# aewallwi/calamity

Measured on AMD Instinct MI355X. Metric: Adam steps/sec (chi2 eval/sec in extra), HERA-350 1024ch DPSS; %HBM roofline, higher is better.
Workload: dtype f32; 1 GPU; hera350: 350 antennas, 61075 baselines x 1024 channels, per-baseline DPSS (sum nvec = 6080554) per time slice, 1 time slice(s), optimizer Adam lr 1e-2, model_regularization none; layout=stream, parallelism=single GPU

## Files before the change

### calamity_amd/csrc/calamity_hip.hip

```cpp
#include "../../include/calamity_hip.h"

#include <hip/hip_runtime.h>
#include <rccl/rccl.h>

#include <algorithm>
#include <cmath>
#include <cstdarg>
#include <cstdio>
#include <cstring>
#include <limits>
#include <map>
#include <memory>
#include <mutex>
#include <numeric>
#include <string>
#include <vector>

#include "fit_kernels.hpp"
#include "dense_kernels.hpp"
#include "split_kernels.hpp"
#include "split2_kernels.hpp"
#include "dense64_kernels.hpp"
#include "multi_mfma_kernels.hpp"
#include "gain_basis_kernels.hpp"
// ... 739 lines not shown
    if (t && nslices > 1) {
      for (int sl = 1; sl < nslices; ++sl)
        if (h_state[sl].t != h_state[0].t)
          return fail(CAL_ERR_STATE, "get_moments: the %d time slices of this solver have applied different numbers of updates (slice 0: %lld, slice %d: %lld); "
                      "one iteration count cannot resume them bit for bit", nslices, (long long)h_state[0].t, sl, (long long)h_state[sl].t);
    }
    if (gm_r) CAL_TRY(download_rows(gm_r, gains_m.as<T>(), nants, 2, 0));
    if (gm_i) CAL_TRY(download_rows(gm_i, gains_m.as<T>(), nants, 2, 1));
    if (gv_r) CAL_TRY(download_rows(gv_r, gains_v.as<T>(), nants, 2, 0));
    if (gv_i) CAL_TRY(download_rows(gv_i, gains_v.as<T>(), nants, 2, 1));
    const size_t cb = (size_t)ncoef * sizeof(T);
    if (cm_r) HIP_TRY(copy_sync(cm_r, coef_m.as<T>(), cb, hipMemcpyDeviceToHost));
    if (cm_i) HIP_TRY(copy_sync(cm_i, coef_m.as<T>() + ncoef, cb, hipMemcpyDeviceToHost));
    if (cv_r) HIP_TRY(copy_sync(cv_r, coef_v.as<T>(), cb, hipMemcpyDeviceToHost));
    if (cv_i) HIP_TRY(copy_sync(cv_i, coef_v.as<T>() + ncoef, cb, hipMemcpyDeviceToHost));
    if (t) *t = h_state->t;
    return CAL_OK;
  }

  int set_moments(const void* gm_r, const void* gm_i, const void* gv_r, const void* gv_i, const void* cm_r, const void* cm_i,
                  const void* cv_r, const void* cv_i, int64_t t) override {
    HIP_TRY(hipSetDevice(device));
    if (!has_problem) return fail(CAL_ERR_STATE, "set_moments before set_problem");
    if (tb_on()) return fail(CAL_ERR_UNSUPPORTED, "set_moments: checkpoint / resume of a fit with a gain time basis is not supported");
    if (gb_on()) return fail(CAL_ERR_UNSUPPORTED, "set_moments: checkpoint / resume of a fit with a gain basis is not supported");
    if (t < 0) return fail(CAL_ERR_INVALID, "set_moments: negative iteration count");
    if (gm_r) CAL_TRY(upload_rows(gm_r, gains_m.as<T>(), nants, 2, 0));
    if (gm_i) CAL_TRY(upload_rows(gm_i, gains_m.as<T>(), nants, 2, 1));
    if (gv_r) CAL_TRY(upload_rows(gv_r, gains_v.as<T>(), nants, 2, 0));
    if (gv_i) CAL_TRY(upload_rows(gv_i, gains_v.as<T>(), nants, 2, 1));
    const size_t cb = (size_t)ncoef * sizeof(T);
    if (cm_r) HIP_TRY(copy_sync(coef_m.as<T>(), cm_r, cb, hipMemcpyHostToDevice));
    if (cm_i) HIP_TRY(copy_sync(coef_m.as<T>() + ncoef, cm_i, cb, hipMemcpyHostToDevice));
    if (cv_r) HIP_TRY(copy_sync(coef_v.as<T>(), cv_r, cb, hipMemcpyHostToDevice));
    if (cv_i) HIP_TRY(copy_sync(coef_v.as<T>() + ncoef, cv_i, cb, hipMemcpyHostToDevice));
    double b1t = 1.0, b2t = 1.0, sched = 1.0;
    for (int64_t k = 0; k < t; ++k) {
      b1t *= opt.beta_1;
      b2t *= opt.beta_2;
    }
    if (opt.optimizer == CAL_OPT_NADAM && t > 0) {
      hipLaunchKernelGGL(nadam_sched_kernel, dim3(1), dim3(1), 0, stream, opt.beta_1, (long long)t, scal.as<double>());
      HIP_TRY(hipGetLastError());
      HIP_TRY(hipMemcpyAsync(&sched, scal.p, sizeof(double), hipMemcpyDeviceToHost, stream));
      HIP_TRY(hipStreamSynchronize(stream));
    }
    for (int sl = 0; sl < nslices; ++sl) {
      h_state[sl].t = t;
      h_state[sl].b1t = b1t;
      h_state[sl].b2t = b2t;
      h_state[sl].nadam_sched = sched;
    }
    return CAL_OK;
  }

  template <typename A> A pass_args() {
    A a{};
    a.data_r = data_r.as<T>();
    a.data_i = data_i.as<T>();
    a.wgts = wgts.as<T>();
    a.gains = gains.as<T2>();
    a.c_r = coef.as<T>();
    a.c_i = coef.as<T>() + ncoef;
    a.q0 = q0.as<T2>();
    a.part = part.as<double>();
    a.state = st_cur();
    a.nslices = nslices;
    a.fpad = fpad;
    a.nbls = nbls;
    return a;
  }
  FusedArgs<T> fused_args() {
    FusedArgs<T> a = pass_args<FusedArgs<T>>();
    a.tiles = tiles.as<T>();
    a.bl_tile = bl_tile.as<long long>();
    a.bl_ant = bl_ant.as<int2>();
    a.items = items.as<Item>();
    a.q1 = q1.as<T2>();
    a.gcp0_r = gcp0.as<T>();
    a.gcp0_i = gcp0.as<T>() + gcp_len;
    a.gcp1_r = gcp1.as<T>();
    a.gcp1_i = gcp1.p ? gcp1.as<T>() + gcp_len : nullptr;
    a.runs = runs.as<int2>();
    a.stream_once = layout == CAL_LAYOUT_STREAM ? 1 : 0;
    a.members = members.as<Member>();
    a.heads = nheads > 0 ? heads.as<int>() : nullptr;
    a.nfreqs = nfreqs;
    return a;
  }
  FusedArgs<T> model_args() {
    FusedArgs<T> a = fused_args();
    a.model_r = model_buf.as<T>();
    a.model_i = model_buf.as<T>() + (size_t)nbls * fpad;
    return a;
  }
  using DenseArgs = typename std::conditional<std::is_same<T, float>::value, MfmaArgs, Dense64Args>::type;
  DenseArgs dense_args() {
    DenseArgs m = pass_args<DenseArgs>();
    m.ops = mf_ops.as<T>();
    m.panels = mf_panels.as<PanelItem>();
    m.gc_r = grad_c0();
    m.gc_i = grad_c0() + ncoef;
    m.slot_map = mf_map.as<int>();
    return m;
  }
  StepShape step_shape(PassAsk ask, int nsteps = 0) const {
    return plan_step(StepInputs{mf_ok, reg == CAL_REG_SUM, reg_prepass, gc_direct, comm_on(), yb_on(), 2LL * nants * fpad + 2LL * ncoef <= (1LL << 20), launch_mode,
                                opt.optimizer == CAL_OPT_LAMB, ask, timing, nsteps >= kGraphMinSteps});
  }

  using FusedFn = void (*)(const FusedArgs<T>);
  static FusedFn pick(bool with_reg, FusedFn reg, FusedFn plain) { return with_reg ? reg : plain; }
  template <int MODE, int L> FusedFn basis_kernel(bool with_reg) const {
    return fold ? pick(with_reg, fused_basis_kernel<T, MODE, true, L, true>, fused_basis_kernel<T, MODE, false, L, true>)
                : pick(with_reg, fused_basis_kernel<T, MODE, true, L, false>, fused_basis_kernel<T, MODE, false, L, false>);
  }
  static constexpr size_t kQLdsMax1 = TileCfg<T, FbSet<T>::fb_min>::q_lds_bytes(false);
  static constexpr size_t kQLdsMax2 = TileCfg<T, FbSet<T>::fb_min>::q_lds_bytes(true);
  template <int MODE> void launch_fused(FusedArgs<T> a, bool with_reg) {
    constexpr bool kPass = MODE == MODE_LOSS || MODE == MODE_GRAD;
    const int nsimple = (kPass && nheads > 0) ? nitems_plain : nitems_simple;
    if (nsimple > 0) {
      FusedFn k = basis_kernel<MODE, kMaxLoads>(with_reg);
      if constexpr (kPass)
        if (small_loads) k = basis_kernel<MODE, kSmallLoads>(with_reg);
      const size_t lds = lds_bytes + (MODE == MODE_GRAD ? (with_reg ? kQLdsMax2 : kQLdsMax1) : 0);
      hipLaunchKernelGGL(k, dim3(nsimple), dim3(kThreads), lds, stream, a);
    }
    if constexpr (kPass) {
      if (nheads > 0) {
        if (nheads_mfma > 0) {
          FusedFn k = pick(with_reg, fused_multi_mfma_kernel<T, MODE, 1>, fused_multi_mfma_kernel<T, MODE, 0>);
          if (with_reg && MODE == MODE_GRAD && heads_one_pass) k = fused_multi_mfma_kernel<T, MODE_GRAD, 2>;
          hipLaunchKernelGGL(k, dim3(mm_grid), dim3(kThreads), lds_multi_mfma_bytes, stream, a);
        }
        if (nheads > nheads_mfma) {
          FusedArgs<T> b = a;
          b.heads = a.heads + mm_grid;
          const FusedFn km = pick(with_reg, fused_multi_kernel<T, MODE, true>, fused_multi_kernel<T, MODE, false>);
          hipLaunchKernelGGL(km, dim3(nheads - nheads_mfma), dim3(kThreads), lds_multi_bytes, stream, b);
        }
      }
    }
    if (nitems > nitems_simple) {
      a.item_base = nitems_simple;
      const FusedFn kg = pick(with_reg, fused_group_kernel<T, MODE, true>, fused_group_kernel<T, MODE, false>);
      hipLaunchKernelGGL(kg, dim3(nitems - nitems_simple), dim3(kThreads), lds_group_bytes, stream, a);
    }
  }
  template <bool GRAD> void launch_dense(const DenseArgs& m) {
    void (*k)(DenseArgs);
    if constexpr (std::is_same<T, float>::value) k = !mf_split ? fused_dense_kernel<GRAD> : mf_split2 ? fused_dense_split2_kernel<GRAD> : fused_dense_split_kernel<GRAD>;
    else k = fused_dense64_kernel<GRAD>;
    hipLaunchKernelGGL(k, dim3(mf_grid), dim3(kDenseThreads), (GRAD ? mf_lds_grad : mf_lds_loss)[0], stream, m);
  }
  T* grad_c0() { return gc_direct ? gcp0.as<T>() : gc0.as<T>(); }
  T* grad_c1() { return gc_direct ? gcp1.as<T>() : gc1.as<T>(); }
  int gain_blocks() const {
    const int cpl = 16 / (int)sizeof(T2) > 0 ? 16 / (int)sizeof(T2) : 1;
    return nants * ((fpad + 64 * cpl - 1) / (64 * cpl));
  }
  template <bool REG> void launch_gain_grad(int blocks, T2* r0, T2* r1, T2* r2, int nants_or_0, int n_parts, const SliceMap& sm) {
    hipLaunchKernelGGL((gain_grad_kernel<T, REG>), dim3(blocks), dim3(256), 0, stream, q0.as<T2>(), q1.as<T2>(), gains.as<T2>(), ant_ptr.as<int>(),
                       ant_ent.as<int2>(), r0, r1, r2, nants_or_0, fpad, part.as<double>(), n_parts, scal.as<double>(), st_cur(), sm);
  }
  void launch_partial_reduce(const DevBuf& gcp, const DevBuf& gc, const SliceMap& sm) {
    hipLaunchKernelGGL(coeff_partial_reduce_kernel<T>, dim3((ncoef + 255) / 256), dim3(256), 0, stream, gcp.as<T>(), gcp.as<T>() + gcp_len, gc.as<T>(),
                       gc.as<T>() + ncoef, coef_grp.as<int>(), grp_coff.as<int>(), grp_item_ptr.as<int>(), item_goff.as<int>(), ncoef, st_cur(), sm);
  }
  PartialSum<T> partial_sum(const DevBuf& gcp) {
    return PartialSum<T>{gcp.as<T>(), gcp.p ? gcp.as<T>() + gcp_len : nullptr, coef_grp.as<int>(), grp_coff.as<int>(), grp_item_ptr.as<int>(), item_goff.as<int>(), ncoef};
  }
  int enqueue_alpha_prepass(int n_parts, const SliceMap& sm) {
    launch_gain_grad<false>(nslices, comm.as<T2>(), comm.as<T2>(), comm.as<T2>(), 0, n_parts, sm);
    if (comm_on()) CAL_TRY(all_reduce(scal.p, 4 * (size_t)nslices, CAL_XCHG_F64, CAL_XCHG_SUM));
    hipLaunchKernelGGL(alpha_kernel, dim3((nslices + 63) / 64), dim3(64), 0, stream, st_cur(), scal.as<double>(), nslices);
    return CAL_OK;
  }
  int time_row() const { return 2 * y_w(); }
  unsigned time_blocks() const { return (unsigned)(((long long)tb_na * (time_row() / (16 / (int)sizeof(T))) + 255) / 256); }
  int enqueue_project(int planes, T2* r0, const SliceMap& sm) {
    const DevState* st = st_cur();
    if (gb_on())
      hipLaunchKernelGGL((gain_project_kernel<T>), dim3(nants, planes), dim3(256), 0, stream, r0, gb_B.as<T>(), (tb_on() ? tb_pf : gb_proj).template as<T>(),
                         nants, fpad, gb_kpad, st, sm);
    if (tb_on()) {
      hipLaunchKernelGGL((gain_time_project_kernel<T>), dim3(time_blocks(), (tb_L + kTimeTile - 1) / kTimeTile, planes), dim3(256), 0, stream,
                         gb_on() ? tb_pf.as<T>() : reinterpret_cast<const T*>(r0), tb_B.as<T>(), gb_proj.as<T>(), tb_na, tb_T, tb_L, tb_lpad, time_row(),
                         (size_t)nants * time_row());
    }
    HIP_TRY(hipGetLastError());
    return CAL_OK;
  }
  int begin_timed_pass(hipEvent_t* end) {
    if (ev_used == ev_pool.size()) {
      hipEvent_t x, y;
      HIP_TRY(hipEventCreate(&x));
      HIP_TRY(hipEventCreate(&y));
// ... 2183 lines not shown
```

### calamity_amd/csrc/check_resources.py

```python
#!/usr/bin/env python3
import re
import sys

cur, bad, seen = None, [], 0
for line in sys.stdin:
    m = re.search(r"remark:\s+Function Name: (\S+)", line)
    if m:
        cur = m.group(1)
        seen += "fused_dense" in cur
        continue
    if cur is not None and "fused_multi_mfma" in cur:
        m = re.search(r"remark:\s+(ScratchSize \[bytes/lane\]|VGPRs Spill|Occupancy \[waves/SIMD\]): (\d+)", line)
        if m and m.group(1).startswith("Occupancy"):
            inst = re.search(r"fused_multi_mfma_kernelI([fd])Li(\d)ELi(\d)E", cur)
            one_wg = inst is None or inst.group(1) == "d" or inst.group(3) == "2"
            if int(m.group(2)) < 2 and not one_wg:
                bad.append(f"{cur}: occupancy {m.group(2)} waves/SIMD (< 2)")
        elif m and int(m.group(2)) != 0:
            bad.append(f"{cur}: {m.group(1)} = {m.group(2)}")
        continue
    if cur is not None and "fused_basis_kernel" in cur:
        m = re.search(r"remark:\s+(ScratchSize \[bytes/lane\]|Occupancy \[waves/SIMD\]): (\d+)", line)
        if m and m.group(1).startswith("Occupancy"):
            if re.search(r"fused_basis_kernelIfLi1ELb0ELi7ELb[01]E", cur) and int(m.group(2)) < 4:
                bad.append(f"{cur}: occupancy {m.group(2)} waves/SIMD (< 4)")
        elif m and int(m.group(2)) != 0:
            bad.append(f"{cur}: {m.group(1)} = {m.group(2)}")
        continue
    if cur is not None and any(k in cur for k in ("gain_project_kernel", "gain_expand_kernel", "gain_time_project_kernel", "gain_time_expand_kernel",
                                             "quality_rows_kernel", "quality_ant_kernel", "robust_rows_kernel", "gain_solve_rows_kernel", "gain_solve_ant_kernel",
                                             "gain_solve_apply_kernel", "coeff_solve_rows_kernel", "coeff_gram_kernel", "coeff_chol_kernel",
                                             "gain_basis_gram_kernel", "gain_basis_chol_kernel", "gain_time_kron_kernel", "gain_time_chol_kernel",
                                             "gain_time_chan_kernel", "fit_error_factor_kernel", "fit_error_leverage_kernel", "fit_error_rows_kernel",
                                             "gn_tangent_rows_kernel", "gn_scale_kernel", "gn_data_kernel", "gn_precond_rows_kernel", "gn_precond_gain_kernel",
                                             "gn_precond_coeff_kernel", "gn_rhs_kernel", "gn_init_kernel", "gn_scalar0_kernel", "gn_diff_kernel",
                                             "gn_scalar1_kernel", "gn_update1_kernel", "gn_scalar2_kernel", "gn_update2_kernel", "gn_apply_kernel",
                                             "gn_round_kernel", "lbfgs_pair_kernel", "lbfgs_reduce_kernel", "lbfgs_coeff_kernel", "lbfgs_direction_kernel",
                                             "lbfgs_trial_kernel", "lbfgs_armijo_kernel", "lbfgs_restore_kernel")):
        m = re.search(r"remark:\s+(ScratchSize \[bytes/lane\]|VGPRs Spill): (\d+)", line)
        if m and int(m.group(2)) != 0:
            bad.append(f"{cur}: {m.group(1)} = {m.group(2)}")
        continue
    if cur is not None and any(k in cur for k in ("dspec_rows_kernel", "dspec_transform_kernel", "dspec_bin_kernel")):
        m = re.search(r"remark:\s+(ScratchSize \[bytes/lane\]|VGPRs Spill|Occupancy \[waves/SIMD\]): (\d+)", line)
        if m and m.group(1).startswith("Occupancy"):
            if "dspec_transform_kernel" in cur and int(m.group(2)) < 2:
                bad.append(f"{cur}: occupancy {m.group(2)} waves/SIMD (< 2)")
        elif m and int(m.group(2)) != 0:
            bad.append(f"{cur}: {m.group(1)} = {m.group(2)}")
        continue
    if cur is not None and any(k in cur for k in ("degen_rows_kernel", "degen_sum_kernel", "degen_solve_kernel", "degen_phase_kernel",
                                             "degen_apply_gains_kernel", "degen_apply_rows_kernel")):
        m = re.search(r"remark:\s+(ScratchSize \[bytes/lane\]|VGPRs Spill): (\d+)", line)
        if m and int(m.group(2)) != 0:
            bad.append(f"{cur}: {m.group(1)} = {m.group(2)}")
        continue
    if cur is None or "fused_dense" not in cur:
        continue
    m = re.search(r"remark:\s+(ScratchSize \[bytes/lane\]|SGPRs Spill|VGPRs Spill|Occupancy \[waves/SIMD\]): (\d+)", line)
    if not m:
        continue
    key, val = m.group(1), int(m.group(2))
    if key.startswith("Occupancy"):
        if val < 2 and "fused_dense_split" not in cur:
            bad.append(f"{cur}: occupancy {val} waves/SIMD (< 2)")
    elif val != 0 and not (key.startswith("SGPRs Spill") and "fused_dense_split" in cur):
        bad.append(f"{cur}: {key} = {val}")
if seen == 0:
    bad.append("no fused_dense kernel found in the compiler's resource remarks")
if bad:
    sys.stderr.write("check_resources: the dense kernels must not spill (scratch traffic breaks their counted waits), the streaming kernel must keep its occupancy:\n  " + "\n  ".join(bad) + "\n")
    sys.exit(1)
print(f"check_resources: {seen} dense kernels, no scratch, no spills")
```

### calamity_amd/csrc/fit_kernels.hpp

```cpp
#pragma once
#include <hip/hip_runtime.h>
#include <stdint.h>

namespace calk {

constexpr int kThreads = 256;
constexpr int kWaves = kThreads / 64;
#ifndef CAL_TILE_LOADS
#define CAL_TILE_LOADS 7
#endif
constexpr int kTileBytes = CAL_TILE_LOADS * 4096;
constexpr int kMaxLoads = kTileBytes / (kThreads * 16);

template <typename T> struct Vec2;
template <> struct Vec2<float> { using type = float2; };
template <> struct Vec2<double> { using type = double2; };
template <typename T> using vec2_t = typename Vec2<T>::type;

struct DevState {
  double loss;
  double prev_loss;
  double min_loss;
  double s_r, s_i;
  double alpha_r, alpha_i;
// ... 6 lines not shown
  int n_recorded;
  int n_recorded_total;
  int done;
  int done_after;
  int improved;
  int record;
  int use_min;
  int reg;
  int nonfinite;
  int nupdates;
  int f32;
  int opt;
  int nesterov;
  double momentum, rho;
  double nadam_sched;
  double ftrl[4];
  double k[6];
};
enum { OPT_ADAM = 0, OPT_ADAMAX = 1, OPT_SGD = 2, OPT_RMSPROP = 3, OPT_ADAGRAD = 4, OPT_NADAM = 5, OPT_ADADELTA = 6, OPT_FTRL = 7, OPT_LAMB = 8 };

struct SliceMap {
  const int* coff;
  const int* part_ptr;
  const int* part_idx;
  int nslices;
  int na_slice;
};
__device__ __forceinline__ int slice_of_coef(const SliceMap& M, int n) {
  int lo = 0, hi = M.nslices - 1;
  while (lo < hi) {
    const int mid = (lo + hi + 1) >> 1;
    if (M.coff[mid] <= n) lo = mid; else hi = mid - 1;
  }
  return lo;
}

struct Item {
  int bl0;
  int tile0, tile1;
  int nvec;
  int coff;
  int goff;
  int fb_log2;
  int role_n;
  long long tile_first;
  int2 ant_first;
  int member0;
  int slice;
};

struct Member {
  int bl;
  int coff;
  int goff;
  int ant0, ant1;
  int slice;
  int item;
  int pad;
};
template <typename T> struct MultiCfg { static constexpr int nb_max = sizeof(T) == 4 ? 8 : 4; };

template <typename T>
struct FusedArgs {
  const T* tiles;
  const long long* bl_tile;
  const int2* bl_ant;
  const T* data_r;
  const T* data_i;
  const T* wgts;
  const vec2_t<T>* gains;
  const T* c_r;
  const T* c_i;
  const Item* items;
  vec2_t<T>* q0;
  vec2_t<T>* q1;
  T* gcp0_r; T* gcp0_i;
  T* gcp1_r; T* gcp1_i;
  double* part;
  T* model_r; T* model_i;
  const DevState* state;
  int nslices;
  int fpad;
  int nbls;
  int stream_once;
  const int2* runs;
  int item_base;
  const Member* members;
  const int* heads;
  int nfreqs;
};

enum { MODE_LOSS = 0, MODE_GRAD = 1, MODE_MODEL = 2, MODE_INIT = 3 };

template <typename T, int FB>
struct TileCfg {
  static constexpr int VEC = 16 / (int)sizeof(T);
  static constexpr int MAXK = kTileBytes / (int)sizeof(T) / FB;
  static constexpr int LPR = FB / VEC;
  static constexpr int NS = kThreads / LPR;
  static constexpr int QT = 1024 / FB;
  static constexpr size_t lds_bytes(bool fold = false) {
    return ((fold ? 4 : 2) * (size_t)kWaves * FB + (fold ? 4 : 2) * (size_t)FB + MAXK) * 2 * sizeof(T)
           + 64;
  }
  static constexpr size_t q_lds_bytes(bool reg) { return (reg ? 2 : 1) * (size_t)1024 * 2 * sizeof(T) + QT * sizeof(long long); }
};

typedef float pair_t __attribute__((ext_vector_type(2)));
__device__ __forceinline__ void pk_fma_lo(pair_t& acc, pair_t a, pair_t b) {
  asm("v_pk_fma_f32 %0, %1, %2, %0 op_sel_hi:[0,1,1]" : "+v"(acc) : "v"(a), "v"(b));
}
__device__ __forceinline__ void pk_fma_hi(pair_t& acc, pair_t a, pair_t b) {
  asm("v_pk_fma_f32 %0, %1, %2, %0 op_sel:[1,0,0] op_sel_hi:[1,1,1]" : "+v"(acc) : "v"(a), "v"(b));
}
__device__ __forceinline__ void fma_rows(float2* acc, const float __attribute__((ext_vector_type(4))) a, const float2 b) {
  const pair_t a01 = {a[0], a[1]}, a23 = {a[2], a[3]}, bb = {b.x, b.y};
  pair_t* p = reinterpret_cast<pair_t*>(acc);
  pk_fma_lo(p[0], a01, bb);
  pk_fma_hi(p[1], a01, bb);
  pk_fma_lo(p[2], a23, bb);
  pk_fma_hi(p[3], a23, bb);
}
__device__ __forceinline__ void fma_cols(float2& acc, const float __attribute__((ext_vector_type(4))) a, const float2* b) {
  const pair_t a01 = {a[0], a[1]}, a23 = {a[2], a[3]};
  pair_t& p = reinterpret_cast<pair_t&>(acc);
  pk_fma_lo(p, a01, pair_t{b[0].x, b[0].y});
  pk_fma_hi(p, a01, pair_t{b[1].x, b[1].y});
  pk_fma_lo(p, a23, pair_t{b[2].x, b[2].y});
  pk_fma_hi(p, a23, pair_t{b[3].x, b[3].y});
}
__device__ __forceinline__ void fma_rows(double2* acc, const double __attribute__((ext_vector_type(2))) a, const double2 b) {
  acc[0].x += a[0] * b.x;
  acc[0].y += a[0] * b.y;
  acc[1].x += a[1] * b.x;
  acc[1].y += a[1] * b.y;
}
__device__ __forceinline__ void fma_cols(double2& acc, const double __attribute__((ext_vector_type(2))) a, const double2* b) {
  acc.x += a[0] * b[0].x + a[1] * b[1].x;
  acc.y += a[0] * b[0].y + a[1] * b[1].y;
}

__device__ __forceinline__ float fma_(float a, float b, float c) { return __builtin_fmaf(a, b, c); }
__device__ __forceinline__ double fma_(double a, double b, double c) { return __builtin_fma(a, b, c); }

__device__ __forceinline__ float pair_sum32(float x) {
  typedef unsigned u2 __attribute__((ext_vector_type(2)));
  const u2 r = __builtin_amdgcn_permlane32_swap(__builtin_bit_cast(unsigned, x), __builtin_bit_cast(unsigned, x), false, false);
  const unsigned a = r[0], b = r[1];
  return __builtin_bit_cast(float, a) + __builtin_bit_cast(float, b);
}
__device__ __forceinline__ float pair_sum16(float x) {
  typedef unsigned u2 __attribute__((ext_vector_type(2)));
  const u2 r = __builtin_amdgcn_permlane16_swap(__builtin_bit_cast(unsigned, x), __builtin_bit_cast(unsigned, x), false, false);
  const unsigned a = r[0], b = r[1];
  return __builtin_bit_cast(float, a) + __builtin_bit_cast(float, b);
}
__device__ __forceinline__ float pair_sum8(float x) {
  const int y = __builtin_amdgcn_update_dpp(0, __builtin_bit_cast(int, x), 0x128, 0xf, 0xf, true);
  return x + __builtin_bit_cast(float, y);
}
__device__ __forceinline__ double pair_sum32(double x) {
  typedef unsigned u2 __attribute__((ext_vector_type(2)));
  const unsigned long long v = __builtin_bit_cast(unsigned long long, x);
  const u2 lo = __builtin_amdgcn_permlane32_swap((unsigned)v, (unsigned)v, false, false);
  const u2 hi = __builtin_amdgcn_permlane32_swap((unsigned)(v >> 32), (unsigned)(v >> 32), false, false);
  const unsigned l0 = lo[0], l1 = lo[1], h0 = hi[0], h1 = hi[1];
  return __builtin_bit_cast(double, ((unsigned long long)h0 << 32) | l0) + __builtin_bit_cast(double, ((unsigned long long)h1 << 32) | l1);
}
__device__ __forceinline__ double pair_sum16(double x) {
  typedef unsigned u2 __attribute__((ext_vector_type(2)));
  const unsigned long long v = __builtin_bit_cast(unsigned long long, x);
  const u2 lo = __builtin_amdgcn_permlane16_swap((unsigned)v, (unsigned)v, false, false);
  const u2 hi = __builtin_amdgcn_permlane16_swap((unsigned)(v >> 32), (unsigned)(v >> 32), false, false);
  const unsigned l0 = lo[0], l1 = lo[1], h0 = hi[0], h1 = hi[1];
  return __builtin_bit_cast(double, ((unsigned long long)h0 << 32) | l0) + __builtin_bit_cast(double, ((unsigned long long)h1 << 32) | l1);
}
__device__ __forceinline__ double pair_sum8(double x) {
  const long long b = __builtin_bit_cast(long long, x);
  const int lo = __builtin_amdgcn_update_dpp(0, (int)b, 0x128, 0xf, 0xf, true);
  const int hi = __builtin_amdgcn_update_dpp(0, (int)(b >> 32), 0x128, 0xf, 0xf, true);
  return x + __builtin_bit_cast(double, ((long long)hi << 32) | (long long)(unsigned)lo);
}
template <int LPR, bool SPLIT = false, typename T> __device__ __forceinline__ T sum_row_lanes(T x) {
  if constexpr (LPR <= 1 && !(SPLIT && LPR == 1)) x += __shfl_xor(x, 1, 64);
  if constexpr (LPR <= 2 && !(SPLIT && LPR == 2)) x += __shfl_xor(x, 2, 64);
  if constexpr (LPR <= 4 && !(SPLIT && LPR == 4)) x += __shfl_xor(x, 4, 64);
  if constexpr (LPR <= 8 && !(SPLIT && LPR == 8)) x = pair_sum8(x);
  if constexpr (LPR <= 16 && !(SPLIT && LPR == 16)) x = pair_sum16(x);
  if constexpr (LPR <= 32 && !(SPLIT && LPR == 32)) x = pair_sum32(x);
  return x;
}

template <typename T> __device__ __forceinline__ T ldsum(T v) {
#pragma unroll
  for (int o = 32; o > 0; o >>= 1) v += __shfl_xor(v, o, 64);
  return v;
}

template <typename T, int FB, int MODE, bool REG, int L = kMaxLoads, bool FOLD = false>
__device__ __forceinline__ void process_item(const FusedArgs<T>& A, const Item it, unsigned char* smem, int item_idx, const DevState* st_own) {
  using C = TileCfg<T, FB>;
  using T2 = vec2_t<T>;
  constexpr int VEC = C::VEC;
  constexpr int LPR = C::LPR;
  constexpr int NS = C::NS;
  constexpr bool FWD = (MODE != MODE_INIT);
  constexpr bool BWD = (MODE == MODE_GRAD || MODE == MODE_INIT);
  const int tid = threadIdx.x;
  const int lane = tid & 63;
  const int wave = tid >> 6;
  const int fq = tid % LPR;
  const int ks = tid / LPR;
  const int f0 = fq * VEC;
  const int nvec = it.nvec;
  constexpr int NP = FOLD ? 2 : 1;
  constexpr int CH = NP * FB;
  const int ntpb = FOLD ? A.nfreqs / (2 * FB) : A.fpad / FB;
  const int tile_elems = nvec * FB;

  T2* s_pv = reinterpret_cast<T2*>(smem);
  T2* s_gv = s_pv + 2 * kWaves * CH;
  T2* s_c = s_gv + 2 * CH;
  T2* s_q = s_c + C::MAXK;
  long long* s_qo = reinterpret_cast<long long*>(s_q + (REG ? 2 : 1) * C::QT * FB);

  typedef T stage_t __attribute__((ext_vector_type(16 / sizeof(T))));

  int own_stop = 0;
  if (st_own) own_stop = st_own->done | st_own->done_after;
  if (FWD) {
    for (int k = tid; k < C::MAXK; k += kThreads) {
      T2 c;
      c.x = k < nvec ? A.c_r[it.coff + k] : (T)0;
      c.y = k < nvec ? A.c_i[it.coff + k] : (T)0;
      s_c[k] = c;
    }
    __syncthreads();
  }
  if (own_stop) return;
  unsigned voff[L];
#pragma unroll
  for (int l = 0; l < L; ++l) voff[l] = (unsigned)((min(l * NS + ks, nvec - 1) * FB + f0) * (int)sizeof(T));
  T2 acc0[L], acc1[L];
#pragma unroll
  for (int l = 0; l < L; ++l) acc0[l].x = acc0[l].y = acc1[l].x = acc1[l].y = 0;
  double loss_acc = 0.0, sr_acc = 0.0, si_acc = 0.0;

  int q_count = 0;
  auto flush_q = [&]() {
    constexpr int kSlotBytes = FB * (int)sizeof(T2);
    typedef unsigned int u4 __attribute__((ext_vector_type(4)));
    for (int b = tid * 16; b < q_count * kSlotBytes; b += kThreads * 16) {
      const int slot = b / kSlotBytes;
      const int within = b - slot * kSlotBytes;
      const long long o = s_qo[slot];
      *reinterpret_cast<u4*>(reinterpret_cast<char*>(A.q0 + o) + within) =
          *reinterpret_cast<const u4*>(reinterpret_cast<const char*>(s_q) + b);
      if (REG)
        *reinterpret_cast<u4*>(reinterpret_cast<char*>(A.q1 + o) + within) =
            *reinterpret_cast<const u4*>(reinterpret_cast<const char*>(s_q + C::QT * FB) + b);
    }
    q_count = 0;
  };

  const long long t_off = it.tile_first;
  const int2 ant = it.ant_first;

  for (int tau = it.tile0; tau < it.tile1; ++tau) {
    const int blrel = tau / ntpb;
    const int fbk = tau - blrel * ntpb;
    const int bl = it.bl0 + blrel;
    if (MODE == MODE_GRAD && q_count == C::QT) flush_q();


    T d_r = 0, d_i = 0, w = 0;
    T2 g0, g1;
    g0.x = g0.y = g1.x = g1.y = 0;
    const int ch = (tid + CH * (tau % (kThreads / CH))) % kThreads;
    const bool hi = FOLD && ch >= FB;
    const int cp = hi ? ch - FB : ch;
    const int col = hi ? A.nfreqs - (fbk + 1) * FB + cp : fbk * FB + cp;
    const long long o_ch = (long long)bl * A.fpad + col;
    if (ch < CH) {
      if (MODE != MODE_MODEL) {
        d_r = __builtin_nontemporal_load(A.data_r + o_ch);
        d_i = __builtin_nontemporal_load(A.data_i + o_ch);
        w = __builtin_nontemporal_load(A.wgts + o_ch);
      }
      if (MODE == MODE_LOSS || MODE == MODE_GRAD) {
        g0 = A.gains[(long long)ant.x * A.fpad + col];
        g1 = A.gains[(long long)ant.y * A.fpad + col];
      }
    }
    const char* src = reinterpret_cast<const char*>(A.tiles + t_off + (long long)fbk * tile_elems);
    stage_t stage[L];
    if (A.stream_once) {
#pragma unroll
      for (int l = 0; l < L; ++l) stage[l] = __builtin_nontemporal_load(reinterpret_cast<const stage_t*>(src + voff[l]));
    } else {
#pragma unroll
      for (int l = 0; l < L; ++l) stage[l] = *reinterpret_cast<const stage_t*>(src + voff[l]);
    }

    T2* pv_par = s_pv + (tau & 1) * kWaves * CH;
    if (FWD) {
      T2 pv[VEC];
#pragma unroll
      for (int u = 0; u < VEC; ++u) pv[u].x = pv[u].y = 0;
#pragma unroll
      for (int l = 0; l < L; ++l) {
        fma_rows(pv, stage[l], s_c[l * NS + ks]);
      }
#pragma unroll
      for (int u = 0; u < VEC; ++u) {
        pv[u].x = sum_row_lanes<LPR, FOLD>(pv[u].x);
        pv[u].y = sum_row_lanes<LPR, FOLD>(pv[u].y);
      }
      if (lane < NP * LPR) {
#pragma unroll
        for (int u = 0; u < VEC; ++u) pv_par[wave * CH + (lane / LPR) * FB + f0 + u] = pv[u];
      }
    }
    __syncthreads();

    if (ch < CH) {
      const int ci = hi ? FB - 1 - cp : cp;
      const int gslot = (hi ? FB : 0) + ci;
      T vr = 0, vi = 0;
      if (FWD) {
        if (FOLD) {
          T orr = 0, oi = 0;
#pragma unroll
          for (int wv = 0; wv < kWaves; ++wv) {
            const T2 e = pv_par[wv * CH + ci];
            const T2 o = pv_par[wv * CH + FB + ci];
            vr += e.x;
            vi += e.y;
            orr += o.x;
            oi += o.y;
          }
          vr = hi ? vr - orr : vr + orr;
          vi = hi ? vi - oi : vi + oi;
        } else {
#pragma unroll
          for (int wv = 0; wv < kWaves; ++wv) {
            const T2 p = pv_par[wv * FB + ch];
            vr += p.x;
            vi += p.y;
          }
        }
      }
      if (MODE == MODE_MODEL) {
        A.model_r[o_ch] = vr;
        A.model_i[o_ch] = vi;
      } else if (MODE == MODE_INIT) {
        const T msk = (fabs(w) <= (T)1e-8) ? (T)0 : (T)1;
        T2 gv;
        gv.x = d_r * msk;
        gv.y = d_i * msk;
        s_gv[gslot] = gv;
      } else {
        const T G_r = g0.x * g1.x + g0.y * g1.y;
        const T G_i = g0.y * g1.x - g0.x * g1.y;
        const T m_r = G_r * vr - G_i * vi;
        const T m_i = G_i * vr + G_r * vi;
        const T r_r = d_r - m_r;
        const T r_i = d_i - m_i;
        loss_acc += (double)(w * (r_r * r_r + r_i * r_i));
        if (REG) {
          sr_acc += (double)(w * m_r);
          si_acc += (double)(w * m_i);
        }
        if (MODE == MODE_GRAD) {
          const T e_r = (T)-2 * w * r_r;
          const T e_i = (T)-2 * w * r_i;
          T2 gv;
          gv.x = G_r * e_r + G_i * e_i;
          gv.y = G_r * e_i - G_i * e_r;
          s_gv[gslot] = gv;
          const int qs = q_count + (hi ? 1 : 0);
          T2 q;
          q.x = vr * e_r + vi * e_i;
          q.y = vr * e_i - vi * e_r;
          s_q[qs * FB + cp] = q;
          if (cp == 0) s_qo[qs] = o_ch;
          if (REG) {
            T2 gw;
            gw.x = G_r * w;
            gw.y = -G_i * w;
            s_gv[CH + gslot] = gw;
            T2 qw;
            qw.x = vr * w;
            qw.y = -vi * w;
            s_q[(C::QT + qs) * FB + cp] = qw;
          }
        }
      }
    }
    if (BWD) {
      __syncthreads();
      T2 gv0[VEC], gv1[VEC];
#pragma unroll
      for (int u = 0; u < VEC; ++u) {
        gv0[u] = s_gv[f0 + u];
        if (REG) gv1[u] = s_gv[CH + f0 + u];
        if (FOLD) {
          const T sg = (ks & 1) ? (T)-1 : (T)1;
          const T2 m0 = s_gv[FB + f0 + u];
          gv0[u].x = fma_(sg, m0.x, gv0[u].x);
          gv0[u].y = fma_(sg, m0.y, gv0[u].y);
          if (REG) {
            const T2 m1 = s_gv[CH + FB + f0 + u];
            gv1[u].x = fma_(sg, m1.x, gv1[u].x);
            gv1[u].y = fma_(sg, m1.y, gv1[u].y);
          }
        }
      }
#pragma unroll
      for (int l = 0; l < L; ++l) {
        fma_cols(acc0[l], stage[l], gv0);
        if (REG) fma_cols(acc1[l], stage[l], gv1);
      }
      if (MODE == MODE_GRAD) q_count += NP;
    }
  }

  if (MODE == MODE_GRAD) {
    __syncthreads();
    flush_q();
  }
  if (MODE == MODE_LOSS || MODE == MODE_GRAD) {
    __syncthreads();
    double* s_red = reinterpret_cast<double*>(s_pv);
    const double l = ldsum(loss_acc);
    const double sr = REG ? ldsum(sr_acc) : 0.0;
    const double si = REG ? ldsum(si_acc) : 0.0;
    if (lane == 0) {
      s_red[wave] = l;
      s_red[kWaves + wave] = sr;
      s_red[2 * kWaves + wave] = si;
    }
    __syncthreads();
    if (tid == 0) {
      double a = 0, b = 0, c = 0;
      for (int wv = 0; wv < kWaves; ++wv) {
        a += s_red[wv];
        b += s_red[kWaves + wv];
        c += s_red[2 * kWaves + wv];
      }
      A.part[(size_t)item_idx * 4 + 0] = a;
      A.part[(size_t)item_idx * 4 + 1] = b;
      A.part[(size_t)item_idx * 4 + 2] = c;
    }
  }
  if (BWD) {
#pragma unroll
    for (int l = 0; l < L; ++l) {
#pragma unroll
      for (int sft = 1; sft < LPR; sft <<= 1) {
        acc0[l].x += __shfl_xor(acc0[l].x, sft, 64);
        acc0[l].y += __shfl_xor(acc0[l].y, sft, 64);
        if (REG) {
          acc1[l].x += __shfl_xor(acc1[l].x, sft, 64);
          acc1[l].y += __shfl_xor(acc1[l].y, sft, 64);
        }
      }
      const int k = l * NS + ks;
      if (fq == 0 && k < nvec) {
        A.gcp0_r[it.goff + k] = acc0[l].x;
        A.gcp0_i[it.goff + k] = acc0[l].y;
        if (REG) {
          A.gcp1_r[it.goff + k] = acc1[l].x;
          A.gcp1_i[it.goff + k] = acc1[l].y;
        }
      }
    }
  }
}

template <typename T, int FB>
constexpr size_t multi_lds_bytes() {
  constexpr int NB = MultiCfg<T>::nb_max;
  return ((size_t)NB * TileCfg<T, FB>::MAXK + (size_t)NB * kWaves * FB + (size_t)NB * FB) * 2 * sizeof(T) + NB * sizeof(Member) + 64;
}
template <typename T, int FB, int MODE, bool REG>
__device__ __forceinline__ void process_multi_item(const FusedArgs<T>& A, const Item it, unsigned char* smem, int item_idx) {
  using C = TileCfg<T, FB>;
  using T2 = vec2_t<T>;
  constexpr int VEC = C::VEC;
  constexpr int LPR = C::LPR;
  constexpr int NS = C::NS;
  constexpr int L = kMaxLoads;
  constexpr int NBMAX = MultiCfg<T>::nb_max;
  constexpr int R = (NBMAX * FB + kThreads - 1) / kThreads;
  constexpr bool GRAD = MODE == MODE_GRAD;
  const int tid = threadIdx.x;
  const int lane = tid & 63;
  const int wave = tid >> 6;
  const int fq = tid % LPR;
  const int ks = tid / LPR;
  const int f0 = fq * VEC;
  const int nvec = it.nvec;
  const int NB = it.role_n >> 2;
  const int ntpb = A.fpad / FB;
  const int tile_elems = nvec * FB;

  T2* s_c = reinterpret_cast<T2*>(smem);
// ... 408 lines not shown
          if (REG) {
            const T2 p2 = s_gvp[kThreads + sb * FB + tid];
            b2.x += p2.x;
            b2.y += p2.y;
          }
        }
        s_gv[tid] = a;
        if (REG) s_gv[FB + tid] = b2;
      }
      __syncthreads();
      T2 gv0[VEC], gv1[VEC];
#pragma unroll
      for (int k = 0; k < VEC; ++k) {
        gv0[k] = s_gv[f0 + k];
        if (REG) gv1[k] = s_gv[FB + f0 + k];
      }
#pragma unroll
      for (int l = 0; l < L; ++l) {
        fma_cols(acc0[l], stage[l], gv0);
        if (REG) fma_cols(acc1[l], stage[l], gv1);
      }
    }
    if (u + 1 < it.tile1 && (u + 1) / ntpb != r) __syncthreads();
  }

  if (MODE == MODE_LOSS || MODE == MODE_GRAD) {
    __syncthreads();
    double* s_red = reinterpret_cast<double*>(s_pv);
    const double l = ldsum(loss_acc);
    const double sr = REG ? ldsum(sr_acc) : 0.0;
    const double si = REG ? ldsum(si_acc) : 0.0;
    if (lane == 0) {
      s_red[wave] = l;
      s_red[kWaves + wave] = sr;
      s_red[2 * kWaves + wave] = si;
    }
    __syncthreads();
    if (tid == 0) {
      double a = 0, b = 0, c = 0;
      for (int wv = 0; wv < kWaves; ++wv) {
        a += s_red[wv];
        b += s_red[kWaves + wv];
        c += s_red[2 * kWaves + wv];
      }
      A.part[(size_t)item_idx * 4 + 0] = a;
      A.part[(size_t)item_idx * 4 + 1] = b;
      A.part[(size_t)item_idx * 4 + 2] = c;
    }
  }
  if (BWD) {
#pragma unroll
    for (int l = 0; l < L; ++l) {
#pragma unroll
      for (int sft = 1; sft < LPR; sft <<= 1) {
        acc0[l].x += __shfl_xor(acc0[l].x, sft, 64);
        acc0[l].y += __shfl_xor(acc0[l].y, sft, 64);
        if (REG) {
          acc1[l].x += __shfl_xor(acc1[l].x, sft, 64);
          acc1[l].y += __shfl_xor(acc1[l].y, sft, 64);
        }
      }
      const int k = l * NS + ks;
      if (fq == 0 && k < nvec) {
        A.gcp0_r[it.goff + k] = acc0[l].x;
        A.gcp0_i[it.goff + k] = acc0[l].y;
        if (REG) {
          A.gcp1_r[it.goff + k] = acc1[l].x;
          A.gcp1_i[it.goff + k] = acc1[l].y;
        }
      }
    }
  }
}

template <typename T, int FB>
constexpr size_t group_lds_bytes() {
  return (2 * (size_t)kWaves * FB + 2 * (size_t)FB + TileCfg<T, FB>::MAXK + 2 * (size_t)kThreads) * 2 * sizeof(T) + kRunMax * sizeof(int2) + 64;
}

#ifndef CAL_WAVES_EU
#define CAL_WAVES_EU 4
#endif
constexpr int kSmallLoads = 2;
template <typename T, int MODE, bool REG, int L = kMaxLoads, bool FOLD = false>
__global__ __launch_bounds__(kThreads) __attribute__((amdgpu_waves_per_eu(L < kMaxLoads ? (sizeof(T) == 4 ? 8 : 6) - (FOLD && REG ? 2 : 0) : ((sizeof(T) == 4 && !REG) ? CAL_WAVES_EU : 1))))
void fused_basis_kernel(const FusedArgs<T> A) {
  extern __shared__ __attribute__((aligned(16))) unsigned char smem[];
  const int idx = A.item_base + blockIdx.x;
  const Item it = A.items[idx];
  const DevState* st_own = nullptr;
  if (A.nslices > 1) st_own = A.state + it.slice;
  else if (A.state->done | A.state->done_after) return;
  if ((MODE == MODE_LOSS || MODE == MODE_GRAD) && (it.role_n & 3) != 0 && A.heads != nullptr) return;
  constexpr int FBM = FbSet<T>::fb_max;
  const int fb = 1 << it.fb_log2;
  if (fb == FBM) process_item<T, FBM, MODE, REG, L, FOLD>(A, it, smem, idx, st_own);
  else if (fb == FBM / 2) process_item<T, FBM / 2, MODE, REG, L, FOLD>(A, it, smem, idx, st_own);
  else if (fb == FBM / 4) process_item<T, FBM / 4, MODE, REG, L, FOLD>(A, it, smem, idx, st_own);
  else if (fb == FBM / 8) process_item<T, FBM / 8, MODE, REG, L, FOLD>(A, it, smem, idx, st_own);
  else process_item<T, FBM / 16, MODE, REG, L, FOLD>(A, it, smem, idx, st_own);
}

template <typename T, int MODE, bool REG>
__global__ __launch_bounds__(kThreads, 2) void fused_multi_kernel(const FusedArgs<T> A) {
  extern __shared__ __attribute__((aligned(16))) unsigned char smem[];
  const int idx = A.heads[blockIdx.x];
  const Item it = A.items[idx];
  if (A.nslices == 1 && (A.state->done | A.state->done_after)) return;
  constexpr int FBM = FbSet<T>::fb_max;
  const int fb = 1 << it.fb_log2;
  if (fb == FBM) process_multi_item<T, FBM, MODE, REG>(A, it, smem, idx);
  else if (fb == FBM / 2) process_multi_item<T, FBM / 2, MODE, REG>(A, it, smem, idx);
  else if (fb == FBM / 4) process_multi_item<T, FBM / 4, MODE, REG>(A, it, smem, idx);
  else if (fb == FBM / 8) process_multi_item<T, FBM / 8, MODE, REG>(A, it, smem, idx);
  else process_multi_item<T, FBM / 16, MODE, REG>(A, it, smem, idx);
}

template <typename T, int MODE, bool REG>
__global__ __launch_bounds__(kThreads) void fused_group_kernel(const FusedArgs<T> A) {
  extern __shared__ __attribute__((aligned(16))) unsigned char smem[];
  const int idx = A.item_base + blockIdx.x;
  const Item it = A.items[idx];
  const DevState* st = A.state;
  if (A.nslices > 1) st += it.slice;
  if (st->done | st->done_after) return;
  constexpr int FBM = FbSet<T>::fb_max;
  const int fb = 1 << it.fb_log2;
  if (fb == FBM) process_group_item<T, FBM, MODE, REG>(A, it, smem, idx);
  else if (fb == FBM / 2) process_group_item<T, FBM / 2, MODE, REG>(A, it, smem, idx);
  else if (fb == FBM / 4) process_group_item<T, FBM / 4, MODE, REG>(A, it, smem, idx);
  else if (fb == FBM / 8) process_group_item<T, FBM / 8, MODE, REG>(A, it, smem, idx);
  else process_group_item<T, FBM / 16, MODE, REG>(A, it, smem, idx);
}

template <typename T>
__global__ void coeff_partial_reduce_kernel(const T* __restrict__ gcp_r, const T* __restrict__ gcp_i, T* __restrict__ gc_r,
                                            T* __restrict__ gc_i, const int* __restrict__ coef_grp,
                                            const int* __restrict__ grp_coff, const int* __restrict__ grp_item_ptr,
                                            const int* __restrict__ item_goff, int ncoef, const DevState* st, const SliceMap M) {
  const int n = blockIdx.x * blockDim.x + threadIdx.x;
  if (n >= ncoef) return;
  if (M.nslices > 1) st += slice_of_coef(M, n);
  if (st->done | st->done_after) return;
  const int g = coef_grp[n];
  const int k = n - grp_coff[g];
  T a = 0, b = 0;
  for (int q = grp_item_ptr[g]; q < grp_item_ptr[g + 1]; ++q) {
    a += gcp_r[item_goff[q] + k];
    b += gcp_i[item_goff[q] + k];
  }
  gc_r[n] = a;
  gc_i[n] = b;
}

__device__ __forceinline__ void sum_partials(const double* __restrict__ part, const int* __restrict__ idx, int p0, int n, const double x[3],
                                             double* sh, double out[3]) {
  const int tid = threadIdx.x;
  double a = 0, b = 0, c = 0;
  if (tid < n) {
    a = x[0];
    b = x[1];
    c = x[2];
  }
  for (int i = tid + 256; i < n; i += 256) {
    const size_t e = idx ? (size_t)idx[p0 + i] : (size_t)(p0 + i);
    a += part[e * 4 + 0];
    b += part[e * 4 + 1];
    c += part[e * 4 + 2];
  }
  a = ldsum(a);
  b = ldsum(b);
  c = ldsum(c);
  if ((tid & 63) == 0) {
    sh[(tid >> 6) * 3 + 0] = a;
    sh[(tid >> 6) * 3 + 1] = b;
    sh[(tid >> 6) * 3 + 2] = c;
  }
  __syncthreads();
  out[0] = ((sh[0] + sh[3]) + sh[6]) + sh[9];
  out[1] = ((sh[1] + sh[4]) + sh[7]) + sh[10];
  out[2] = ((sh[2] + sh[5]) + sh[8]) + sh[11];
}
__device__ __forceinline__ void slice_partials(const SliceMap& M, int t, int nparts, const double* __restrict__ part, int& p0, int& n, double x[3]) {
// ... 838 lines not shown
```

Before: 359.3 steps/s.

## Issue first tile loads before coefficient staging and template the non-temporal hint

Measured after the change: 362.2 steps/s, median of 2. About the same (+0.8%).

```diff
diff --git a/calamity_amd/csrc/calamity_hip.hip b/calamity_amd/csrc/calamity_hip.hip
--- a/calamity_amd/csrc/calamity_hip.hip
+++ b/calamity_amd/csrc/calamity_hip.hip
@@ -845,7 +845,6 @@
     a.gcp1_r = gcp1.as<T>();
     a.gcp1_i = gcp1.p ? gcp1.as<T>() + gcp_len : nullptr;
     a.runs = runs.as<int2>();
-    a.stream_once = layout == CAL_LAYOUT_STREAM ? 1 : 0;
     a.members = members.as<Member>();
     a.heads = nheads > 0 ? heads.as<int>() : nullptr;
     a.nfreqs = nfreqs;
@@ -875,8 +874,9 @@
   using FusedFn = void (*)(const FusedArgs<T>);
   static FusedFn pick(bool with_reg, FusedFn reg, FusedFn plain) { return with_reg ? reg : plain; }
   template <int MODE, int L> FusedFn basis_kernel(bool with_reg) const {
-    return fold ? pick(with_reg, fused_basis_kernel<T, MODE, true, L, true>, fused_basis_kernel<T, MODE, false, L, true>)
-                : pick(with_reg, fused_basis_kernel<T, MODE, true, L, false>, fused_basis_kernel<T, MODE, false, L, false>);
+    if (fold) return pick(with_reg, fused_basis_kernel<T, MODE, true, L, true, true>, fused_basis_kernel<T, MODE, false, L, true, true>);
+    return layout == CAL_LAYOUT_STREAM ? pick(with_reg, fused_basis_kernel<T, MODE, true, L, false, true>, fused_basis_kernel<T, MODE, false, L, false, true>)
+                                       : pick(with_reg, fused_basis_kernel<T, MODE, true, L, false, false>, fused_basis_kernel<T, MODE, false, L, false, false>);
   }
   static constexpr size_t kQLdsMax1 = TileCfg<T, FbSet<T>::fb_min>::q_lds_bytes(false);
   static constexpr size_t kQLdsMax2 = TileCfg<T, FbSet<T>::fb_min>::q_lds_bytes(true);
diff --git a/calamity_amd/csrc/check_resources.py b/calamity_amd/csrc/check_resources.py
--- a/calamity_amd/csrc/check_resources.py
+++ b/calamity_amd/csrc/check_resources.py
@@ -22,7 +22,7 @@
     if cur is not None and "fused_basis_kernel" in cur:
         m = re.search(r"remark:\s+(ScratchSize \[bytes/lane\]|Occupancy \[waves/SIMD\]): (\d+)", line)
         if m and m.group(1).startswith("Occupancy"):
-            if re.search(r"fused_basis_kernelIfLi1ELb0ELi7ELb[01]E", cur) and int(m.group(2)) < 4:
+            if re.search(r"fused_basis_kernelIfLi1ELb0ELi7ELb[01]ELb[01]EE", cur) and int(m.group(2)) < 4:
                 bad.append(f"{cur}: occupancy {m.group(2)} waves/SIMD (< 4)")
         elif m and int(m.group(2)) != 0:
             bad.append(f"{cur}: {m.group(1)} = {m.group(2)}")
diff --git a/calamity_amd/csrc/check_stream_loads.py b/calamity_amd/csrc/check_stream_loads.py
--- /dev/null
+++ b/calamity_amd/csrc/check_stream_loads.py
@@ -0,0 +1,50 @@
+#!/usr/bin/env python3
+import re
+import sys
+
+NAME = re.compile(r"^(_ZN4calk18fused_basis_kernelI([fd])Li(\d)ELb([01])ELi(\d+)ELb([01])ELb([01])EE\w*):")
+
+
+def main(path):
+    counts, cur = {}, None
+    with open(path) as f:
+        for line in f:
+            m = NAME.match(line)
+            if m:
+                cur = m.group(1)
+                counts[cur] = dict(dtype=m.group(2), mode=int(m.group(3)), loads=int(m.group(5)), nt_inst=m.group(7) == "1", nt=0, plain=0)
+                continue
+            if cur is None:
+                continue
+            if line.startswith(".Lfunc_end"):
+                cur = None
+                continue
+            text = line.split(";")[0].split()
+            if text and text[0] == "global_load_dwordx4":
+                counts[cur]["nt" if "nt" in text[1:] else "plain"] += 1
+    bad = []
+    for name, c in counts.items():
+        gains16 = c["dtype"] == "d" and c["mode"] in (0, 1)
+        if c["nt_inst"]:
+            want_plain = 2 * c["nt"] // c["loads"] if gains16 else 0
+            if c["nt"] == 0 or c["nt"] % c["loads"] != 0:
+                bad.append(f"{name}: a STREAM instance with {c['nt']} non-temporal 16-byte loads (a positive multiple of L = {c['loads']} expected)")
+            if c["plain"] != want_plain:
+                bad.append(f"{name}: a STREAM instance with {c['plain']} plain 16-byte loads beside {c['nt']} non-temporal ones ({want_plain} expected): a tile load lost its hint")
+        else:
+            if c["nt"] != 0:
+                bad.append(f"{name}: a SHARED instance with {c['nt']} non-temporal 16-byte loads (its tiles are re-used)")
+            if c["plain"] == 0:
+                bad.append(f"{name}: no 16-byte load found")
+    n_nt = sum(c["nt_inst"] for c in counts.values())
+    if n_nt == 0 or n_nt == len(counts):
+        bad.append(f"{len(counts)} instances of fused_basis_kernel found, {n_nt} of them STREAM: both kinds are expected")
+    if bad:
+        sys.stderr.write("check_stream_loads:\n  " + "\n  ".join(bad) + "\n")
+        return 1
+    print(f"check_stream_loads: {len(counts)} instances of fused_basis_kernel, {n_nt} with non-temporal tile loads, {len(counts) - n_nt} with plain ones")
+    return 0
+
+
+if __name__ == "__main__":
+    sys.exit(main(sys.argv[1]))
diff --git a/calamity_amd/csrc/fit_kernels.hpp b/calamity_amd/csrc/fit_kernels.hpp
--- a/calamity_amd/csrc/fit_kernels.hpp
+++ b/calamity_amd/csrc/fit_kernels.hpp
@@ -112,7 +112,6 @@
   int nslices;
   int fpad;
   int nbls;
-  int stream_once;
   const int2* runs;
   int item_base;
   const Member* members;
@@ -227,7 +226,7 @@
   return v;
 }
 
-template <typename T, int FB, int MODE, bool REG, int L = kMaxLoads, bool FOLD = false>
+template <typename T, int FB, int MODE, bool REG, int L = kMaxLoads, bool FOLD = false, bool NT = FOLD>
 __device__ __forceinline__ void process_item(const FusedArgs<T>& A, const Item it, unsigned char* smem, int item_idx, const DevState* st_own) {
   using C = TileCfg<T, FB>;
   using T2 = vec2_t<T>;
@@ -236,6 +235,7 @@
   constexpr int NS = C::NS;
   constexpr bool FWD = (MODE != MODE_INIT);
   constexpr bool BWD = (MODE == MODE_GRAD || MODE == MODE_INIT);
+  constexpr bool EARLY = !(sizeof(T) == 4 && MODE == MODE_GRAD && REG && L < kMaxLoads && !FOLD);
   const int tid = threadIdx.x;
   const int lane = tid & 63;
   const int wave = tid >> 6;
@@ -258,19 +258,73 @@
 
   int own_stop = 0;
   if (st_own) own_stop = st_own->done | st_own->done_after;
+  constexpr int NK = L * NS;
+  constexpr int NC = (NK + kThreads - 1) / kThreads;
+  T2 c_pre[NC];
   if (FWD) {
-    for (int k = tid; k < C::MAXK; k += kThreads) {
-      T2 c;
-      c.x = k < nvec ? A.c_r[it.coff + k] : (T)0;
-      c.y = k < nvec ? A.c_i[it.coff + k] : (T)0;
-      s_c[k] = c;
+#pragma unroll
+    for (int j = 0; j < NC; ++j) {
+      const int k = min(tid + j * kThreads, nvec - 1);
+      c_pre[j].x = A.c_r[it.coff + k];
+      c_pre[j].y = A.c_i[it.coff + k];
+    }
+  }
+  unsigned voff[L];
+#pragma unroll
+  for (int l = 0; l < L; ++l) voff[l] = (unsigned)((min(l * NS + ks, nvec - 1) * FB + f0) * (int)sizeof(T));
+
+  const long long t_off = it.tile_first;
+  const int2 ant = it.ant_first;
+
+  int ch = 0, cp = 0;
+  bool hi = false;
+  long long o_ch = 0;
+  T d_r = 0, d_i = 0, w = 0;
+  T2 g0, g1;
+  g0.x = g0.y = g1.x = g1.y = 0;
+  stage_t stage[L];
+  auto issue = [&](const int tau) {
+    const int blrel = tau / ntpb;
+    const int fbk = tau - blrel * ntpb;
+    const int bl = it.bl0 + blrel;
+    d_r = d_i = w = 0;
+    g0.x = g0.y = g1.x = g1.y = 0;
+    ch = (tid + CH * (tau % (kThreads / CH))) % kThreads;
+    hi = FOLD && ch >= FB;
+    cp = hi ? ch - FB : ch;
+    const int col = hi ? A.nfreqs - (fbk + 1) * FB + cp : fbk * FB + cp;
+    o_ch = (long long)bl * A.fpad + col;
+    if (ch < CH) {
+      if (MODE != MODE_MODEL) {
+        d_r = __builtin_nontemporal_load(A.data_r + o_ch);
+        d_i = __builtin_nontemporal_load(A.data_i + o_ch);
+        w = __builtin_nontemporal_load(A.wgts + o_ch);
+      }
+      if (MODE == MODE_LOSS || MODE == MODE_GRAD) {
+        g0 = A.gains[(long long)ant.x * A.fpad + col];
+        g1 = A.gains[(long long)ant.y * A.fpad + col];
+      }
+    }
+    const char* src = reinterpret_cast<const char*>(A.tiles + t_off + (long long)fbk * tile_elems);
+#pragma unroll
+    for (int l = 0; l < L; ++l) {
+      const stage_t* p = reinterpret_cast<const stage_t*>(src + voff[l]);
+      if constexpr (NT) stage[l] = __builtin_nontemporal_load(p);
+      else stage[l] = *p;
+    }
+  };
+  if constexpr (EARLY) issue(it.tile0);
+  if (FWD) {
+#pragma unroll
+    for (int j = 0; j < NC; ++j) {
+      const int k = tid + j * kThreads;
+      T2 c = c_pre[j];
+      if (k >= nvec) c.x = c.y = (T)0;
+      if (NK % kThreads == 0 || k < NK) s_c[k] = c;
     }
     __syncthreads();
   }
   if (own_stop) return;
-  unsigned voff[L];
-#pragma unroll
-  for (int l = 0; l < L; ++l) voff[l] = (unsigned)((min(l * NS + ks, nvec - 1) * FB + f0) * (int)sizeof(T));
   T2 acc0[L], acc1[L];
 #pragma unroll
   for (int l = 0; l < L; ++l) acc0[l].x = acc0[l].y = acc1[l].x = acc1[l].y = 0;
@@ -293,45 +347,7 @@
     q_count = 0;
   };
 
-  const long long t_off = it.tile_first;
-  const int2 ant = it.ant_first;
-
-  for (int tau = it.tile0; tau < it.tile1; ++tau) {
-    const int blrel = tau / ntpb;
-    const int fbk = tau - blrel * ntpb;
-    const int bl = it.bl0 + blrel;
-    if (MODE == MODE_GRAD && q_count == C::QT) flush_q();
-
-
-    T d_r = 0, d_i = 0, w = 0;
-    T2 g0, g1;
-    g0.x = g0.y = g1.x = g1.y = 0;
-    const int ch = (tid + CH * (tau % (kThreads / CH))) % kThreads;
-    const bool hi = FOLD && ch >= FB;
-    const int cp = hi ? ch - FB : ch;
-    const int col = hi ? A.nfreqs - (fbk + 1) * FB + cp : fbk * FB + cp;
-    const long long o_ch = (long long)bl * A.fpad + col;
-    if (ch < CH) {
-      if (MODE != MODE_MODEL) {
-        d_r = __builtin_nontemporal_load(A.data_r + o_ch);
-        d_i = __builtin_nontemporal_load(A.data_i + o_ch);
-        w = __builtin_nontemporal_load(A.wgts + o_ch);
-      }
-      if (MODE == MODE_LOSS || MODE == MODE_GRAD) {
-        g0 = A.gains[(long long)ant.x * A.fpad + col];
-        g1 = A.gains[(long long)ant.y * A.fpad + col];
-      }
-    }
-    const char* src = reinterpret_cast<const char*>(A.tiles + t_off + (long long)fbk * tile_elems);
-    stage_t stage[L];
-    if (A.stream_once) {
-#pragma unroll
-      for (int l = 0; l < L; ++l) stage[l] = __builtin_nontemporal_load(reinterpret_cast<const stage_t*>(src + voff[l]));
-    } else {
-#pragma unroll
-      for (int l = 0; l < L; ++l) stage[l] = *reinterpret_cast<const stage_t*>(src + voff[l]);
-    }
-
+  auto consume = [&](const int tau) {
     T2* pv_par = s_pv + (tau & 1) * kWaves * CH;
     if (FWD) {
       T2 pv[VEC];
@@ -453,6 +469,12 @@
       }
       if (MODE == MODE_GRAD) q_count += NP;
     }
+  };
+  if constexpr (EARLY) consume(it.tile0);
+  for (int tau = it.tile0 + (EARLY ? 1 : 0); tau < it.tile1; ++tau) {
+    if (MODE == MODE_GRAD && q_count == C::QT) flush_q();
+    issue(tau);
+    consume(tau);
   }
 
   if (MODE == MODE_GRAD) {
@@ -1027,8 +1049,8 @@
 #define CAL_WAVES_EU 4
 #endif
 constexpr int kSmallLoads = 2;
-template <typename T, int MODE, bool REG, int L = kMaxLoads, bool FOLD = false>
-__global__ __launch_bounds__(kThreads) __attribute__((amdgpu_waves_per_eu(L < kMaxLoads ? (sizeof(T) == 4 ? 8 : 6) - (FOLD && REG ? 2 : 0) : ((sizeof(T) == 4 && !REG) ? CAL_WAVES_EU : 1))))
+template <typename T, int MODE, bool REG, int L = kMaxLoads, bool FOLD = false, bool NT = FOLD>
+__global__ __launch_bounds__(kThreads) __attribute__((amdgpu_waves_per_eu(L < kMaxLoads ? (sizeof(T) == 4 ? 8 : 6) - (FOLD && REG ? 2 : 0) : ((sizeof(T) == 4 && !REG) ? CAL_WAVES_EU : (sizeof(T) == 8 && MODE == MODE_GRAD) ? ((REG || FOLD) ? 3 : 4) : 1))))
 void fused_basis_kernel(const FusedArgs<T> A) {
   extern __shared__ __attribute__((aligned(16))) unsigned char smem[];
   const int idx = A.item_base + blockIdx.x;
@@ -1039,11 +1061,11 @@
   if ((MODE == MODE_LOSS || MODE == MODE_GRAD) && (it.role_n & 3) != 0 && A.heads != nullptr) return;
   constexpr int FBM = FbSet<T>::fb_max;
   const int fb = 1 << it.fb_log2;
-  if (fb == FBM) process_item<T, FBM, MODE, REG, L, FOLD>(A, it, smem, idx, st_own);
-  else if (fb == FBM / 2) process_item<T, FBM / 2, MODE, REG, L, FOLD>(A, it, smem, idx, st_own);
-  else if (fb == FBM / 4) process_item<T, FBM / 4, MODE, REG, L, FOLD>(A, it, smem, idx, st_own);
-  else if (fb == FBM / 8) process_item<T, FBM / 8, MODE, REG, L, FOLD>(A, it, smem, idx, st_own);
-  else process_item<T, FBM / 16, MODE, REG, L, FOLD>(A, it, smem, idx, st_own);
+  if (fb == FBM) process_item<T, FBM, MODE, REG, L, FOLD, NT>(A, it, smem, idx, st_own);
+  else if (fb == FBM / 2) process_item<T, FBM / 2, MODE, REG, L, FOLD, NT>(A, it, smem, idx, st_own);
+  else if (fb == FBM / 4) process_item<T, FBM / 4, MODE, REG, L, FOLD, NT>(A, it, smem, idx, st_own);
+  else if (fb == FBM / 8) process_item<T, FBM / 8, MODE, REG, L, FOLD, NT>(A, it, smem, idx, st_own);
+  else process_item<T, FBM / 16, MODE, REG, L, FOLD, NT>(A, it, smem, idx, st_own);
 }
 
 template <typename T, int MODE, bool REG>
```
